# lxd99/TPNet

Measured on NVIDIA B200. Metric: temporal edges/sec (update+pairwise encode), higher is better.
Workload: dtype f32

## Files before the change

tpnet_b200/csrc/tpn_update.cu:

```cuda
#include <stdlib.h>

#include "tpn_common.cuh"
#include "tpn_radix.cuh"

namespace tpn {

namespace {

int g_debug_flags = 0;
thread_local int g_dev_slot = 0;

constexpr int kSmallMaxMsgs = 4096;
constexpr int kRankMaxMsgs = 1024;
constexpr int kPrepThreads = 1024;
constexpr int kWalkThreads = 256;
constexpr int kHubMin = 64;
constexpr int kGiantMin = 2048;
constexpr int kHubConsumers = 4;
constexpr int kHubThreads = (kHubConsumers + 1) * 32;
constexpr int kHubStages = 4;
constexpr int kHubSlotFloats = kHubConsumers * 32;
constexpr int kHubMetaChunk = 512;
constexpr int kChunkMin = 256;
constexpr size_t kSnapMaxBytes = (size_t)8 << 30;
constexpr int kSmallWalkThreads = 256;
constexpr int kHub2Producers = 7;
constexpr int kHub2Threads = (1 + kHub2Producers) * 32;
constexpr int kHub2SlotFloats = 64;
#ifndef TPN_HUB2_GIANT_FLOATS
#define TPN_HUB2_GIANT_FLOATS 16
#endif
constexpr int kHub2GiantFloats = TPN_HUB2_GIANT_FLOATS;
static_assert(kHub2GiantFloats == 8 || kHub2GiantFloats == 16 || kHub2GiantFloats == 32, "giant slices are 32, 64 or 128 bytes");
constexpr int kGiantLs = kHub2GiantFloats == 8 ? 1 : (kHub2GiantFloats == 16 ? 2 : 3);
constexpr int kGiantSpm = 16 >> kGiantLs;
constexpr int kGiantSpmMax = kGiantSpm > 4 ? kGiantSpm : 4;
constexpr int kHub2Stages = kHub2Producers + 4;
constexpr int kCtrGiant = 0, kCtrHub = 1, kCtrWork0 = 2, kCtrSmall = 6, kCtrHub2Work = 7, kCtrHub2Giant = 8;
constexpr int kCtrChunks = 9;
constexpr int kCtrStream = 10, kCtrStreamBlocks = 11, kCtrStreamProd = 12, kCtrStreamActive = 13, kCtrStreamChain = 14, kCtrStreamTicket = 15;
constexpr int kStreamSlice = kHub2GiantFloats;
constexpr int kStreamBlock = 32 * kGiantSpm;
constexpr uint32_t kNoPart = 0xffffffffu;
constexpr int kCtrSmClaim = 16;
constexpr int kCtrSlots = kCtrSmClaim + 256;
constexpr int kBarWords = 32;

struct DecayArgs {
    float c[TPN_MAX_LAYERS];
    int has_decay;
};

constexpr uint32_t kDirect = 0x80000000u;

struct MsgSource {
    const long long* a;
    const long long* b;
    const double* t;
    long long B;
    long long direct_from;
    __device__ __forceinline__ void get(int m, long long& tgt, long long& oth, int& widx) const {
        if (B > 0) {
            const int j = m < B ? m : (int)(m - B);
            tgt = m < B ? a[j] : b[j];
            oth = m < B ? b[j] : a[j];
            widx = j;
        } else {
            tgt = a[m];
            oth = b[m];
            widx = m;
        }
    }
};

struct Workspace {
    float* w;
    uint32_t* key_a;
    uint32_t* key_b;
    uint32_t* val_a;
    uint32_t* val_b;
    uint32_t* ssrc;
    float* sw;
    uint32_t* hist;
    uint32_t* hist2;
    uint32_t* bar;
    uint32_t* sslot;
    uint32_t* slen;
    float* snap;
    uint32_t* hub_giant;
    uint32_t* hub_reg;
    uint32_t* ctr;
    uint32_t* small_heads;
    uint32_t* hub_len;
    uint32_t* hub_part;
    uint32_t* giant_cbase;
    float* partial;
    int* svst;
    float* gprod;
    uint32_t* gflag;
    uint32_t* gblk;
    bool has_snap;
    bool has_stream;
    size_t bytes;
};

inline size_t snap_bytes(size_t E, int num_layer, int64_t row_stride) {
    return sizeof(float) * E * (size_t)num_layer * (size_t)row_stride;
}

inline size_t align_up(size_t x, size_t a) { return (x + a - 1) / a * a; }

constexpr size_t kStreamMaxBytes = (size_t)4 << 30;
constexpr int kGiantSortMaxC = 2048;
inline int stream_slices(int num_layer, int64_t row_stride) {
    return num_layer * (int)((row_stride + kStreamSlice - 1) / kStreamSlice);
}
inline size_t stream_prod_bytes(size_t E, int num_layer, int64_t row_stride) {
    return sizeof(float) * E * (size_t)stream_slices(num_layer, row_stride) * kStreamSlice + 256;
}
inline size_t stream_flag_words(size_t E) { return E / kStreamBlock + E / kGiantMin + 4; }

Workspace carve(void* base, int64_t batch, int num_layer, int64_t row_stride) {
    const size_t E = 2 * (size_t)batch;
    const size_t nblk = (E + kRadixTile - 1) / kRadixTile;
    char* p = reinterpret_cast<char*>(base);
    size_t off = 0;
    Workspace ws;
    auto take = [&](size_t bytes) { char* r = p ? p + off : nullptr; off += align_up(bytes, 256); return r; };
    ws.w = reinterpret_cast<float*>(take(sizeof(float) * E));
    ws.key_a = reinterpret_cast<uint32_t*>(take(4 * E));
    ws.key_b = reinterpret_cast<uint32_t*>(take(4 * E));
    ws.val_a = reinterpret_cast<uint32_t*>(take(4 * E));
    ws.val_b = reinterpret_cast<uint32_t*>(take(4 * E));
    ws.ssrc = reinterpret_cast<uint32_t*>(take(4 * E));
    ws.sw = reinterpret_cast<float*>(take(4 * E));
    ws.hist = reinterpret_cast<uint32_t*>(take(4 * kRadixBins * (nblk + 1)));
    ws.hist2 = reinterpret_cast<uint32_t*>(take(4 * kRadixBins * (nblk + 1)));
    ws.bar = reinterpret_cast<uint32_t*>(take(4 * kBarWords));
    ws.sslot = reinterpret_cast<uint32_t*>(take(4 * E));
    ws.slen = reinterpret_cast<uint32_t*>(take(4 * E));
    ws.has_snap = snap_bytes(E, num_layer, row_stride) <= kSnapMaxBytes;
    ws.snap = reinterpret_cast<float*>(take((ws.has_snap ? snap_bytes(E, num_layer, row_stride) : 0) + 16));
    ws.hub_giant = reinterpret_cast<uint32_t*>(take(4 * (E / kGiantMin + 2)));
    const size_t hub_cap = E / kHubMin + E / kChunkMin + E / kGiantMin + 4;
    const size_t part_rows = E / kChunkMin + E / kGiantMin + 2;
    ws.hub_reg = reinterpret_cast<uint32_t*>(take(4 * hub_cap));
    ws.hub_len = reinterpret_cast<uint32_t*>(take(4 * hub_cap));
    ws.hub_part = reinterpret_cast<uint32_t*>(take(4 * hub_cap));
    ws.giant_cbase = reinterpret_cast<uint32_t*>(take(4 * (E / kGiantMin + 2)));
    ws.partial = reinterpret_cast<float*>(take(ws.has_snap ? 4 * part_rows * (size_t)num_layer * (size_t)row_stride : 16));
    ws.ctr = reinterpret_cast<uint32_t*>(take(4 * kCtrSlots));
    ws.small_heads = reinterpret_cast<uint32_t*>(take(4 * E));
    ws.svst = reinterpret_cast<int*>(take(4 * (E + 4) * (size_t)(num_layer > 1 ? num_layer - 1 : 1) + 16));
    ws.gflag = reinterpret_cast<uint32_t*>(take(4 * stream_flag_words(E)));
    ws.gblk = reinterpret_cast<uint32_t*>(take(4 * (kGiantSortMaxC + 1)));
    ws.has_stream = ws.has_snap && stream_prod_bytes(E, num_layer, row_stride) <= kStreamMaxBytes &&
                    E / kGiantMin + 2 <= (size_t)kGiantSortMaxC;
    ws.gprod = reinterpret_cast<float*>(take(ws.has_stream ? stream_prod_bytes(E, num_layer, row_stride) : 16));
    ws.bytes = off;
    return ws;
}

__device__ __forceinline__ float edge_weight(double t, float t_last_f, float neg_lambda) {
    const float diff = __fsub_rn(t_last_f, (float)t);
    const float arg = __fmul_rn(neg_lambda, diff);
    return (float)exp((double)arg);
}

struct SweepArgs {
    long long total4;
    int ds4;
};

__device__ __forceinline__ void sweep_body(const StateView& st, const DecayArgs& decay, long long total4, int ds4,
                                           long long first, long long stride) {
    const long long per_node4 = (long long)st.num_layer * ds4;
    for (long long i = first; i < total4; i += stride) {
        const long long node = i / per_node4;
        const int r = (int)(i - node * per_node4);
        const int li = r / ds4;
        float* p = st.data + node * st.node_stride + st.row_stride + (long long)r * 4;
        float4 x = ld4(p);
        scale4(x, decay.c[li]);
        st4(p, x);
    }
}

__global__ void __launch_bounds__(kPrepThreads)
prep_small_kernel(MsgSource msgs, int E, float t_last_f, float neg_lambda, long long num_nodes,
                  uint32_t* __restrict__ skey, uint32_t* __restrict__ ssrc, float* __restrict__ sw,
                  uint32_t* __restrict__ sslot, uint32_t* __restrict__ slen, int* __restrict__ err_flag,
                  double* decay_log, int L, long long new_epoch, DecayArgs decay, StateView st, SweepArgs sweep) {
    if (blockIdx.x > 0) {
        sweep_body(st, decay, sweep.total4, sweep.ds4, (long long)(blockIdx.x - 1) * kPrepThreads + threadIdx.x,
                   (long long)(gridDim.x - 1) * kPrepThreads);
        return;
    }
    __shared__ __align__(16) unsigned long long comp[kSmallMaxMsgs];
    __shared__ float wsm[kSmallMaxMsgs];
    const int n_w = msgs.B > 0 ? (int)msgs.B : E;
    const bool message_mode = msgs.B == 0;
    const bool lazy = decay_log != nullptr;
    if (threadIdx.x == 0 && decay_log != nullptr && decay.has_decay) {
        for (int l = 0; l < L; ++l) decay_log[new_epoch * L + l] = decay_log[(new_epoch - 1) * L + l] * (double)decay.c[l];
    }
    if (E <= kRankMaxMsgs) {
        uint32_t* c32 = reinterpret_cast<uint32_t*>(comp);
        const bool narrow = num_nodes < (1ll << 22);
        const int Epad = (E + 3) & ~3;
        for (int m = threadIdx.x; m < Epad; m += kPrepThreads) {
            uint32_t key = 0xffffffffu >> 10;
            if (m < E) {
                long long tgt, oth;
                int widx;
                msgs.get(m, tgt, oth, widx);
                const bool ok = tgt >= 0 && tgt < num_nodes && oth >= 0 && oth < num_nodes;
                if (!ok && err_flag != nullptr) *err_flag = 1;
                key = ok ? (uint32_t)tgt : (uint32_t)num_nodes;
                if (m < n_w) wsm[m] = edge_weight(msgs.t[m], t_last_f, neg_lambda);
            }
            if (narrow) c32[m] = (key << 10) | (uint32_t)m;
            else comp[m] = ((unsigned long long)(m < E ? key : 0xffffffffu) << 32) | (uint32_t)m;
        }
// ... 42 lines not shown
            sw[rank] = wsm[j];
            sslot[rank] = (uint32_t)slot;
            slen[rank] = (uint32_t)(upper - lower);
        }
        return;
    }
    int P = 1;
    while (P < E) P <<= 1;
    for (int m = threadIdx.x; m < P; m += kPrepThreads) {
        unsigned long long c = ~0ull;
        if (m < E) {
            long long tgt, oth;
            int widx;
            msgs.get(m, tgt, oth, widx);
            const bool ok = tgt >= 0 && tgt < num_nodes && oth >= 0 && oth < num_nodes;
            if (!ok && err_flag != nullptr) *err_flag = 1;
            const uint32_t key = ok ? (uint32_t)tgt : (uint32_t)num_nodes;
            c = ((unsigned long long)key << 32) | (uint32_t)m;
            if (m < n_w) wsm[m] = edge_weight(msgs.t[m], t_last_f, neg_lambda);
        }
        comp[m] = c;
    }
    __syncthreads();
    for (int k = 2; k <= P; k <<= 1) {
        for (int j = k >> 1; j > 0; j >>= 1) {
            for (int i = threadIdx.x; i < P; i += kPrepThreads) {
                const int ixj = i ^ j;
                if (ixj > i) {
                    const unsigned long long a = comp[i], b = comp[ixj];
                    const bool up = (i & k) == 0;
                    if ((a > b) == up) { comp[i] = b; comp[ixj] = a; }
                }
            }
            __syncthreads();
        }
    }
    for (int p = threadIdx.x; p < E; p += kPrepThreads) {
        const unsigned long long c = comp[p];
        const uint32_t m = (uint32_t)c;
        const uint32_t mykey = (uint32_t)(c >> 32);
        long long tgt_unused, oth;
        int j;
        msgs.get((int)m, tgt_unused, oth, j);
        const uint32_t other = (uint32_t)oth;
        skey[p] = mykey;
        ssrc[p] = other;
        sw[p] = wsm[j];
        const unsigned long long other_lo = (unsigned long long)other << 32;
        const unsigned long long next_lo = (unsigned long long)(mykey + 1) << 32;
        int lo = 0, hi = E;
        while (lo < hi) {
            const int mid = (lo + hi) >> 1;
            if (comp[mid] < other_lo) lo = mid + 1; else hi = mid;
        }
        uint32_t slot = (uint32_t)lo;
        if (message_mode && (lo >= E || (uint32_t)(comp[lo] >> 32) != other)) {
            if (lazy && (long long)other < msgs.direct_from && err_flag != nullptr) *err_flag = 2;
            slot = kDirect;
        }
        sslot[p] = slot;
        lo = p; hi = E;
        while (lo < hi) {
            const int mid = (lo + hi) >> 1;
            if (comp[mid] < next_lo) lo = mid + 1; else hi = mid;
        }
        slen[p] = (uint32_t)(lo - p);
    }
}

struct PrepArgs {
    MsgSource msgs;
    Count count;
    float t_last_f, neg_lambda;
    long long num_nodes;
    float* w;
    uint32_t* key;
    uint32_t* val;
    int* err_flag;
    double* decay_log;
    int L;
    long long new_epoch;
    DecayArgs decay;
    uint32_t* ctr;
};

__device__ __forceinline__ void prep_body(const PrepArgs& a, int m) {
    if (m == 0 && a.decay_log != nullptr && a.decay.has_decay) {
        for (int l = 0; l < a.L; ++l)
            a.decay_log[a.new_epoch * a.L + l] = a.decay_log[(a.new_epoch - 1) * a.L + l] * (double)a.decay.c[l];
    }
    if (m < kCtrSlots) a.ctr[m] = 0;
    if (m == 0 && a.count.dev != nullptr && *a.count.dev > a.count.cap && a.err_flag != nullptr) *a.err_flag = 4;
    const int E = a.count.get();
    if (m >= E) return;
    long long tgt, oth;
    int widx;
    a.msgs.get(m, tgt, oth, widx);
    const bool ok = tgt >= 0 && tgt < a.num_nodes && oth >= 0 && oth < a.num_nodes;
    if (!ok && a.err_flag != nullptr) *a.err_flag = 1;
    const int n_w = a.msgs.B > 0 ? (int)a.msgs.B : E;
    if (m < n_w) a.w[m] = edge_weight(a.msgs.t[m], a.t_last_f, a.neg_lambda);
    a.key[m] = ok ? (uint32_t)tgt : (uint32_t)a.num_nodes;
    a.val[m] = (uint32_t)m;
}

__global__ void __launch_bounds__(256) prep_large_kernel(PrepArgs a) {
    prep_body(a, blockIdx.x * blockDim.x + threadIdx.x);
}

struct PayloadArgs {
    const uint32_t* order;
    const uint32_t* skey;
    uint32_t* key_out;
    MsgSource msgs;
    const float* w;
    Count count;
    uint32_t* ssrc;
    float* sw;
    uint32_t* sslot;
    uint32_t* slen;
    uint32_t* hub_giant;
    uint32_t* hub_reg;
    uint32_t* small_heads;
    uint32_t* ctr;
    int* svst;
    const int* stamps;
    int L, E4;
    long long num_nodes;
    int* err_flag;
    uint32_t* hub_len;
    uint32_t* hub_part;
    uint32_t* giant_cbase;
    int chunk;
};

__device__ __forceinline__ void payload_body(const PayloadArgs& a, int p) {
    const uint32_t* __restrict__ order = a.order;
    const uint32_t* __restrict__ skey = a.skey;
    const MsgSource& msgs = a.msgs;
    const float* __restrict__ w = a.w;
    const int E = a.count.get();
    uint32_t* __restrict__ ssrc = a.ssrc;
    float* __restrict__ sw = a.sw;
    uint32_t* __restrict__ sslot = a.sslot;
    uint32_t* __restrict__ slen = a.slen;
    uint32_t* __restrict__ hub_giant = a.hub_giant;
    uint32_t* __restrict__ hub_reg = a.hub_reg;
    uint32_t* __restrict__ small_heads = a.small_heads;
    uint32_t* __restrict__ ctr = a.ctr;
    int* __restrict__ svst = a.svst;
    const int* __restrict__ stamps = a.stamps;
    const int L = a.L, E4 = a.E4;
    const long long num_nodes = a.num_nodes;
    int* __restrict__ err_flag = a.err_flag;
    const int lane = threadIdx.x & 31;
    bool small_head = false;
    if (p < E) {
        const uint32_t m = order[p];
        long long tgt_unused, oth;
        int j;
        msgs.get((int)m, tgt_unused, oth, j);
        const uint32_t other = (uint32_t)oth;
        const uint32_t mykey = skey[p];
        if (a.key_out != skey) a.key_out[p] = mykey;
        ssrc[p] = other;
        float wv = w[j];
        if (sslot != nullptr) {
            int lo = 0, hi = E;
            while (lo < hi) {
                const int mid = (lo + hi) >> 1;
                if (skey[mid] < other) lo = mid + 1; else hi = mid;
            }
            uint32_t slot = (uint32_t)lo;
            if (msgs.B == 0 && (lo >= E || skey[lo] != other)) {
                if (stamps != nullptr && (long long)other < msgs.direct_from && err_flag != nullptr) *err_flag = 2;
                slot = kDirect;
                wv = __int_as_float(__float_as_int(wv) | 0x80000000);
            }
            sslot[p] = slot;
        }
        sw[p] = wv;
        uint32_t len = 0;
        if (p == 0 || skey[p - 1] != mykey) {
            int lo = p, hi = E;
            while (lo < hi) {
                const int mid = (lo + hi) >> 1;
                if (skey[mid] <= mykey) lo = mid + 1; else hi = mid;
            }
            len = (uint32_t)(lo - p);
            if ((long long)mykey < num_nodes) {
                if (len >= (uint32_t)kGiantMin) {
                    const uint32_t gi = atomicAdd(&ctr[kCtrGiant], 1u);
                    hub_giant[gi] = (uint32_t)p;
                    if (a.chunk > 0) {
                        const uint32_t nch = (len + (uint32_t)a.chunk - 1u) / (uint32_t)a.chunk;
                        const uint32_t cb = atomicAdd(&ctr[kCtrChunks], nch);
                        const uint32_t eb = atomicAdd(&ctr[kCtrHub], nch);
                        a.giant_cbase[gi] = cb;
                        for (uint32_t c = 0; c < nch; ++c) {
                            hub_reg[eb + c] = (uint32_t)p + c * (uint32_t)a.chunk;
                            a.hub_len[eb + c] = min((uint32_t)a.chunk, len - c * (uint32_t)a.chunk);
                            a.hub_part[eb + c] = cb + c;
                        }
                    }
                } else if (len >= (uint32_t)kHubMin) {
                    const uint32_t e = atomicAdd(&ctr[kCtrHub], 1u);
                    hub_reg[e] = (uint32_t)p;
                    a.hub_len[e] = len;
                    a.hub_part[e] = kNoPart;
                } else {
                    small_head = true;
                }
            }
        }
        slen[p] = len;
        if (svst != nullptr) {
            for (int l = 0; l < L - 1; ++l)
                svst[(size_t)l * E4 + p] = (long long)other < num_nodes ? stamps[(long long)other * L + l] : -1;
        }
    }
    const uint32_t mask = __ballot_sync(0xffffffffu, small_head);
    if (mask != 0) {
        const int leader = __ffs(mask) - 1;
        uint32_t base = 0;
        if (lane == leader) base = atomicAdd(&ctr[kCtrSmall], (uint32_t)__popc(mask));
        base = __shfl_sync(0xffffffffu, base, leader);
        if (small_head) small_heads[base + __popc(mask & ((1u << lane) - 1u))] = (uint32_t)p;
    }
}

__global__ void __launch_bounds__(256) payload_kernel(PayloadArgs a) {
    payload_body(a, blockIdx.x * blockDim.x + threadIdx.x);
}

constexpr int kGiantSortMax = kGiantSortMaxC;
struct GiantSmem {
    uint32_t head_s[kGiantSortMax], len_s[kGiantSortMax], sorted_s[kGiantSortMax];
};
__device__ __forceinline__ void sort_giants_body(GiantSmem& sm, uint32_t* __restrict__ hub_giant,
                                                 const uint32_t* __restrict__ slen, uint32_t* __restrict__ ctr,
                                                 uint32_t* __restrict__ gblk, uint32_t* __restrict__ gflag, Count count,
                                                 int stream_mode) {
    const uint32_t stream_min = stream_mode == 0 ? 0u
                                : (stream_mode == 2 ? (uint32_t)kGiantMin
                                                    : max((uint32_t)kGiantMin, (uint32_t)(count.get() >> 2)));
    const int n = (int)ctr[kCtrGiant];
    if (n < 1 || n > kGiantSortMax) return;
    for (int i = threadIdx.x; i < n; i += blockDim.x) {
        sm.head_s[i] = hub_giant[i];
        sm.len_s[i] = slen[sm.head_s[i]];
    }
    __syncthreads();
    for (int i = threadIdx.x; i < n; i += blockDim.x) {
        const uint32_t li = sm.len_s[i];
        int rank = 0;
        for (int j = 0; j < n; ++j) rank += (sm.len_s[j] > li || (sm.len_s[j] == li && j < i)) ? 1 : 0;
        hub_giant[rank] = sm.head_s[i];
        sm.sorted_s[rank] = li;
    }
    __syncthreads();
    if (threadIdx.x == 0 && stream_min > 0) {
        uint32_t blocks = 0;
        int ns = 0;
        for (; ns < n && sm.sorted_s[ns] >= stream_min; ++ns) {
            gblk[ns] = blocks;
            blocks += (sm.sorted_s[ns] + (uint32_t)kStreamBlock - 1u) / (uint32_t)kStreamBlock;
        }
        gblk[ns] = blocks;
        ctr[kCtrStream] = (uint32_t)ns;
        ctr[kCtrStreamBlocks] = blocks;
        sm.head_s[0] = blocks;
    }
    __syncthreads();
    if (stream_min > 0) {
        const uint32_t blocks = sm.head_s[0];
        for (uint32_t i = threadIdx.x; i < blocks; i += blockDim.x) gflag[i] = 0;
    }
}
__global__ void __launch_bounds__(1024)
sort_giants_kernel(uint32_t* __restrict__ hub_giant, const uint32_t* __restrict__ slen, uint32_t* __restrict__ ctr,
                   uint32_t* __restrict__ gblk, uint32_t* __restrict__ gflag, Count count, int stream_mode) {
    __shared__ GiantSmem sm;
    sort_giants_body(sm, hub_giant, slen, ctr, gblk, gflag, count, stream_mode);
}

struct FrontArgs {
    PrepArgs prep;
    uint32_t *key_a, *key_b, *val_a, *val_b, *hist, *hist2, *bar;
    int passes;
};

__device__ __forceinline__ void grid_barrier(uint32_t* bar, uint32_t& target, int* err_flag) {
    __syncthreads();
    if (threadIdx.x == 0) {
        target += gridDim.x;
        __threadfence();
        atomicAdd(bar, 1u);
        uint32_t seen;
        long long spins = 0;
        do {
            asm volatile("ld.acquire.gpu.global.u32 %0, [%1];" : "=r"(seen) : "l"(bar) : "memory");
            if (seen >= target) break;
            if (++spins > (1ll << 22)) {
                if (err_flag != nullptr) *err_flag = 8;
                break;
            }
        } while (true);
    }
    __syncthreads();
}

union FrontSmem {
    uint32_t bins[kRadixBins];
    ScatterSmem scatter;
};
// ... 93 lines not shown

    float* tbase = st.data + (long long)key * st.node_stride + (long long)(ALL ? 1 : layer) * st.row_stride;
    float4 acc[V];
#pragma unroll
    for (int k = 0; k < V; ++k) {
        const int c = col0 + k * 32;
        const int tli = ALL ? (c < span4 ? c / ds4 : 0) : layer - 1;
        long long tstamp = 0;
        if (LAZY && c < span4) tstamp = st.stamps[(long long)key * L + tli];
        acc[k] = (c < span4 && tstamp >= 0) ? ld4(tbase + 4 * (long long)c) : make_float4(0.f, 0.f, 0.f, 0.f);
        if (LAZY && c < span4 && tstamp >= 0) scale4(acc[k], decay_factor(st, tli, tstamp));
    }

    for (int base = 0; base < len; base += 32) {
        const int nmsg = min(32, len - base);
        uint32_t my_v = 0, my_slot = 0;
        float my_w = 0.f;
        long long my_vstamp = 0;
        if (lane < nmsg) {
            const int p = wid + base + lane;
            my_v = ssrc[p];
            my_w = sw[p];
            if (ALL) my_slot = sslot[p];
            else if (LAZY && layer >= 2) my_vstamp = st.stamps[(long long)my_v * L + (layer - 2)];
        }
        for (int j0 = 0; j0 < nmsg; j0 += D) {
            float4 x[D][V];
            float w[D];
            long long vstamp[D];
#pragma unroll
            for (int j = 0; j < D; ++j) {
                const int jj = j0 + j;
                const int sl = jj < nmsg ? jj : 0;
                const uint32_t v = __shfl_sync(0xffffffffu, my_v, sl);
                w[j] = __shfl_sync(0xffffffffu, my_w, sl);
                const uint32_t slot = ALL ? __shfl_sync(0xffffffffu, my_slot, sl) : 0u;
                vstamp[j] = (!ALL && LAZY) ? __shfl_sync(0xffffffffu, my_vstamp, sl) : 0;
                const float* sstate = st.data + (long long)v * st.node_stride +
                                      (long long)(ALL ? 0 : layer - 1) * st.row_stride;
                const bool direct = ALL && (slot & kDirect) != 0;
                const float* ssnap = ALL ? snap + (long long)(slot & ~kDirect) * snap4 * 4 : nullptr;
#pragma unroll
                for (int k = 0; k < V; ++k) {
                    const int c = col0 + k * 32;
                    float4 val = make_float4(0.f, 0.f, 0.f, 0.f);
                    if (jj < nmsg && c < span4) {
                        if (ALL) {
                            val = (c < soff || direct) ? ld4(sstate + 4 * (long long)c)
                                                       : ld4(ssnap + 4 * (long long)(c - soff));
                            if (LAZY && direct && c >= ds4) {
                                const int sli = c / ds4 - 1;
                                const int sst = st.stamps[(long long)v * L + sli];
                                if (sst >= 0) scale4(val, decay_factor(st, sli, sst));
                            }
                        }
                        else if (vstamp[j] >= 0) val = ld4(sstate + 4 * (long long)c);
                    }
                    x[j][k] = val;
                }
            }
#pragma unroll
            for (int j = 0; j < D; ++j) {
                if (j0 + j < nmsg) {
                    if (!ALL && LAZY && layer >= 2 && vstamp[j] >= 0) {
                        const float f = decay_factor(st, layer - 2, vstamp[j]);
#pragma unroll
                        for (int k = 0; k < V; ++k) scale4(x[j][k], f);
                    }
#pragma unroll
                    for (int k = 0; k < V; ++k) axpy4_rn(acc[k], x[j][k], w[j]);
                }
            }
        }
    }
#pragma unroll
    for (int k = 0; k < V; ++k) {
        const int c = col0 + k * 32;
        if (c < span4) st4(tbase + 4 * (long long)c, acc[k]);
    }
    if (LAZY && write_stamp && lane == 0) st.stamps[(long long)key * L + (layer - 1)] = (int)st.epoch;
}

template <bool LAZY>
__global__ void __launch_bounds__(256)
snapshot_kernel(StateView st, const uint32_t* __restrict__ skey, Count count, int ds4, float* __restrict__ snap,
                int srow0) {
    const int p = (blockIdx.x * 256 + threadIdx.x) >> 5;
    const int lane = threadIdx.x & 31;
    if (p >= count.get()) return;
    const uint32_t key = skey[p];
    if ((long long)key >= st.num_nodes) return;
    if (p > 0 && skey[p - 1] == key) return;
    const int L = st.num_layer;
    const int snap4 = (L - srow0) * ds4;
    const float* rows = st.data + (long long)key * st.node_stride + (long long)srow0 * st.row_stride;
    float* slot = snap + (long long)p * snap4 * 4;
    float fmine = 1.0f;
    if (LAZY && lane < L - srow0 && srow0 + lane >= 1) {
        const int li = srow0 + lane - 1;
        const long long stamp = st.stamps[(long long)key * L + li];
        fmine = stamp >= 0 ? decay_factor(st, li, stamp) : -1.0f;
    }
    float f[TPN_MAX_LAYERS];
#pragma unroll
    for (int l = 0; l < TPN_MAX_LAYERS; ++l) f[l] = LAZY ? __shfl_sync(0xffffffffu, fmine, l) : 1.0f;
    for (int c0 = lane; c0 < snap4; c0 += 128) {
        float4 v[4];
        float fk[4];
#pragma unroll
        for (int k = 0; k < 4; ++k) {
            const int c = c0 + 32 * k;
            const int li = c / ds4;
            fk[k] = li == 0 ? f[0] : (li == 1 ? f[1] : (li == 2 ? f[2] : f[3]));
            v[k] = (c < snap4 && fk[k] >= 0.f) ? ld4(rows + 4 * (long long)c) : make_float4(0.f, 0.f, 0.f, 0.f);
        }
#pragma unroll
        for (int k = 0; k < 4; ++k) {
            const int c = c0 + 32 * k;
            if (c < snap4) {
                if (LAZY && fk[k] >= 0.f && fk[k] != 1.0f) scale4(v[k], fk[k]);
                st4(slot + 4 * (long long)c, v[k]);
            }
        }
    }
}

__global__ void __launch_bounds__(256)
stamp_targets_kernel(StateView st, int layer, const uint32_t* __restrict__ skey, Count count) {
    const int p = blockIdx.x * blockDim.x + threadIdx.x;
    if (p >= count.get()) return;
    const uint32_t key = skey[p];
    if ((long long)key >= st.num_nodes) return;
    if (p > 0 && skey[p - 1] == key) return;
    if (layer >= 1) {
        st.stamps[(long long)key * st.num_layer + (layer - 1)] = (int)st.epoch;
    } else {
        for (int l = 0; l < st.num_layer; ++l) st.stamps[(long long)key * st.num_layer + l] = (int)st.epoch;
    }
}


struct HubSmem {
    float ring[kHubStages][32][kHubSlotFloats];
    float wring[kHubStages][32];
    int vring[kHubStages][32];
    uint32_t msrc[2][kHubMetaChunk + 4];
    float mw[2][kHubMetaChunk + 4];
    uint32_t mx[2][kHubMetaChunk + 4];
    uint64_t full[kHubStages];
    uint64_t empty[kHubStages];
    uint64_t mfull[2];
    int item[4];
};

template <bool LAZY, bool ALL>
__global__ void __launch_bounds__(kHubThreads)
walk_hub_kernel(StateView st, int layer, const uint32_t* __restrict__ skey, const uint32_t* __restrict__ ssrc,
                const float* __restrict__ sw, const uint32_t* __restrict__ xarr, const uint32_t* __restrict__ slen,
                const float* __restrict__ snap, const uint32_t* __restrict__ hub_giant,
                const uint32_t* __restrict__ hub_reg, uint32_t* __restrict__ ctr, int work_ctr, int span,
                int slice_w, int slices, DecayArgs dnow) {
    extern __shared__ __align__(128) unsigned char hub_raw[];
    HubSmem& sm = *reinterpret_cast<HubSmem*>(hub_raw);
    const int warp = threadIdx.x >> 5;
    const int lane = threadIdx.x & 31;
    const int L = st.num_layer;
    const int rs = (int)st.row_stride;
    const bool has_x = ALL || (LAZY && layer >= 2);
    if (threadIdx.x == 0) {
        for (int i = 0; i < kHubStages; ++i) {
            mbar_init(&sm.full[i], 1);
            mbar_init(&sm.empty[i], kHubConsumers);
        }
        mbar_init(&sm.mfull[0], 1);
        mbar_init(&sm.mfull[1], 1);
        asm volatile("fence.mbarrier_init.release.cluster;" ::: "memory");
    }
    __syncthreads();
    const uint32_t n_giant = ctr[0], n_reg = ctr[1];
    const uint32_t total = (n_giant + n_reg) * (uint32_t)slices;
    uint32_t blk = 0;
    uint32_t mit = 0;
    for (;;) {
        if (threadIdx.x == 0) sm.item[0] = (int)atomicAdd(&ctr[work_ctr], 1u);
        __syncthreads();
        const uint32_t work = (uint32_t)sm.item[0];
        __syncthreads();
        if (work >= total) break;
        const uint32_t it = work / (uint32_t)slices;
        const int slice = (int)(work - it * (uint32_t)slices);
        const int head = (int)(it < n_giant ? hub_giant[it] : hub_reg[it - n_giant]);
        const int len = (int)slen[head];
        const uint32_t key = skey[head];
        const int c0 = slice * slice_w;
        const int c1 = min(span, c0 + slice_w);
        const uint32_t msg_bytes = (uint32_t)(c1 - c0) * 4u;

        if (warp == kHubConsumers) {
            const int nchunk = (len + kHubMetaChunk - 1) / kHubMetaChunk;
            auto issue_meta = [&](int c, uint32_t m) {
                const int cs = c * kHubMetaChunk;
                const int cn = min(kHubMetaChunk, len - cs);
                const int a0 = (head + cs) & ~3;
                const uint32_t bytes = (uint32_t)(((head + cs + cn) - a0 + 3) & ~3) * 4u;
                const int buf = (int)(m & 1u);
                fence_proxy_async_smem();
// ... 1040 lines not shown
    const bool lazy = st->stamps != nullptr;
    const int L = st->num_layer;

    DecayArgs dargs;
    dargs.has_decay = 0;
    for (int l = 0; l < TPN_MAX_LAYERS; ++l) dargs.c[l] = 1.0f;
    if (decay != nullptr) {
        bool all_one = true;
        for (int l = 0; l < L; ++l) {
            dargs.c[l] = decay[l];
            all_one = all_one && decay[l] == 1.0f;
        }
        dargs.has_decay = all_one ? 0 : 1;
    }
    long long new_epoch = st->epoch;
    double new_floor = st->cum_floor;
    if (lazy && dargs.has_decay) {
        if (st->epoch + 1 >= st->log_capacity) return TPN_ERR_LOG_FULL;
        double cmin = 1.0;
        for (int l = 0; l < L; ++l) cmin = dargs.c[l] < cmin ? (double)dargs.c[l] : cmin;
        new_floor = (st->epoch == 0 ? 1.0 : st->cum_floor);
        if (st->epoch > 0 && !(new_floor * cmin >= 1e-200)) return TPN_ERR_LOG_FULL;
        new_floor *= cmin;
        new_epoch = st->epoch + 1;
    }

    const int ds4 = (int)(st->row_stride / 4);
    const float t_last_f = (float)t_last;
    double* log_w = lazy ? st->decay_log : nullptr;
    const bool force_per_layer = (g_debug_flags & TPN_DEBUG_PER_LAYER_WALK) != 0;
    const bool snapshot_path = ws.has_snap && !(force_per_layer && !(count_dev == nullptr && E <= kSmallMaxMsgs));
    const bool small_path = count_dev == nullptr && E <= kSmallMaxMsgs;
    const bool hubs = !small_path;
    const int E4 = (E + 3) & ~3;
    const bool eager_sweep = !lazy && dargs.has_decay;
    int chunk = st->giant_chunk > 0 ? (int)st->giant_chunk : 0;
    if (chunk > 0 && chunk < kChunkMin) chunk = kChunkMin;
    if (chunk > kGiantMin) chunk = kGiantMin;
    chunk &= ~31;
    const long long sweep_total4 = st->num_nodes * (long long)L * ds4;
    const int stream_mode = (ws.has_stream && chunk == 0 && (g_debug_flags & TPN_DEBUG_NO_STREAM) == 0)
                                ? ((g_debug_flags & TPN_DEBUG_STREAM_ALL) ? 2 : 1) : 0;

    StateView view = make_view(st);
    view.epoch = new_epoch;

    const bool do_front = phase != TPN_UPDATE_APPLY;
    const bool do_rest = phase != TPN_UPDATE_PREPARE;
    const bool snap_early = lazy && !small_path;
    if (small_path) {
        if (phase == TPN_UPDATE_PREPARE) return TPN_OK;
        SweepArgs sw_args;
        sw_args.total4 = eager_sweep ? sweep_total4 : 0;
        sw_args.ds4 = ds4;
        unsigned grid = 1;
        if (eager_sweep) {
            const long long want = (sweep_total4 + kPrepThreads - 1) / kPrepThreads;
            const long long cap = (long long)device_sm_count() * 4;
            grid += (unsigned)(want < cap ? (want < 1 ? 1 : want) : cap);
        }
        prep_small_kernel<<<grid, kPrepThreads, 0, stream>>>(msgs, E, t_last_f, neg_lambda, st->num_nodes, ws.key_a,
                                                             ws.ssrc, ws.sw, ws.sslot, ws.slen, err_flag_dev, log_w, L,
                                                             new_epoch, dargs, view, sw_args);
    } else if (do_front) {
        int bits = 0;
        while ((1ll << bits) <= st->num_nodes) ++bits;
        const int passes = (bits + 7) / 8;
        const int nblk = (E + kRadixTile - 1) / kRadixTile;
        struct { PrepArgs prep; PayloadArgs pay; } fa;
        fa.prep.msgs = msgs;
        fa.prep.count = cnt;
        fa.prep.t_last_f = t_last_f;
        fa.prep.neg_lambda = neg_lambda;
        fa.prep.num_nodes = st->num_nodes;
        fa.prep.w = ws.w;
        fa.prep.key = ws.key_a;
        fa.prep.val = ws.val_a;
        fa.prep.err_flag = err_flag_dev;
        fa.prep.decay_log = log_w;
        fa.prep.L = L;
        fa.prep.new_epoch = new_epoch;
        fa.prep.decay = dargs;
        fa.prep.ctr = ws.ctr;
        fa.pay.order = nullptr;
        fa.pay.skey = nullptr;
        fa.pay.key_out = ws.key_a;
        fa.pay.msgs = msgs;
        fa.pay.w = ws.w;
        fa.pay.count = cnt;
        fa.pay.ssrc = ws.ssrc;
        fa.pay.sw = ws.sw;
        fa.pay.sslot = snapshot_path ? ws.sslot : nullptr;
        fa.pay.slen = ws.slen;
        fa.pay.hub_giant = ws.hub_giant;
        fa.pay.hub_reg = ws.hub_reg;
        fa.pay.small_heads = ws.small_heads;
        fa.pay.ctr = ws.ctr;
        fa.pay.svst = (lazy && !snapshot_path && L >= 2) ? ws.svst : nullptr;
        fa.pay.stamps = st->stamps;
        fa.pay.L = L;
        fa.pay.E4 = E4;
        fa.pay.num_nodes = st->num_nodes;
        fa.pay.err_flag = err_flag_dev;
        fa.pay.hub_len = ws.hub_len;
        fa.pay.hub_part = ws.hub_part;
        fa.pay.giant_cbase = ws.giant_cbase;
        fa.pay.chunk = (snapshot_path && hubs) ? chunk : 0;
        const bool fused_front = (g_debug_flags & TPN_DEBUG_LEGACY_FRONT) == 0 && front_kernel_ok();
        if (fused_front) {
            FrontArgs fr;
            fr.prep = fa.prep;
            fr.key_a = ws.key_a; fr.key_b = ws.key_b; fr.val_a = ws.val_a; fr.val_b = ws.val_b;
            fr.hist = ws.hist; fr.hist2 = ws.hist2; fr.bar = ws.bar;
            fr.passes = passes;
            const int sms = device_sm_count();
            const unsigned grid = (unsigned)(nblk < 1 ? 1 : (nblk < sms ? nblk : sms));
            void* kargs[] = {&fr};
            if (cudaMemsetAsync(ws.bar, 0, 4 * kBarWords, stream) != cudaSuccess ||
                cudaLaunchCooperativeKernel((const void*)front_kernel, dim3(grid), dim3(kRadixThreads), kargs, 0,
                                            stream) != cudaSuccess) {
                set_cuda_error(cudaGetLastError());
                return TPN_ERR_CUDA;
            }
            const bool odd = (passes & 1) != 0;
            fa.pay.order = odd ? ws.val_b : ws.val_a;
            fa.pay.skey = odd ? ws.key_b : ws.key_a;
            payload_kernel<<<(E + 255) / 256, 256, 0, stream>>>(fa.pay);
            if (snapshot_path && chunk == 0) {
                sort_giants_kernel<<<1, 1024, 0, stream>>>(ws.hub_giant, ws.slen, ws.ctr, ws.gblk, ws.gflag, cnt, stream_mode);
            }
        } else
        {
            prep_large_kernel<<<(unsigned)((E + 255) / 256 < 2 ? 2 : (E + 255) / 256), 256, 0, stream>>>(fa.prep);
            uint32_t *kin = ws.key_a, *kout = ws.key_b, *vin = ws.val_a, *vout = ws.val_b;
            for (int p = 0; p < passes; ++p) {
                radix_hist_kernel<<<nblk, kRadixThreads, 0, stream>>>(kin, cnt, 8 * p, ws.hist);
                const int prefixed = (nblk > kRadixDirectBlocks || count_dev != nullptr) ? 1 : 0;
                if (prefixed) radix_prefix_kernel<<<kRadixBins / 8, 256, 0, stream>>>(ws.hist, cnt);
                radix_scatter_kernel<<<nblk, kRadixThreads, 0, stream>>>(kin, vin, kout, vout, cnt, 8 * p, ws.hist,
                                                                         prefixed);
                uint32_t* tk = kin; kin = kout; kout = tk;
                uint32_t* tv = vin; vin = vout; vout = tv;
            }
            fa.pay.order = vin;
            fa.pay.skey = kin;
            payload_kernel<<<(E + 255) / 256, 256, 0, stream>>>(fa.pay);
            if (snapshot_path && chunk == 0) {
                sort_giants_kernel<<<1, 1024, 0, stream>>>(ws.hub_giant, ws.slen, ws.ctr, ws.gblk, ws.gflag, cnt, stream_mode);
            }
        }
    }
    if (!small_path && do_rest && eager_sweep) {
        const long long want = (sweep_total4 + 255) / 256;
        const long long cap = (long long)device_sm_count() * 16;
        const unsigned grid = (unsigned)(want < cap ? (want < 1 ? 1 : want) : cap);
        sweep_decay_kernel<<<grid, 256, 0, stream>>>(view, dargs, sweep_total4, ds4);
    }

    const int srow0 = (g_debug_flags & TPN_DEBUG_SNAPSHOT_P0) ? 0 : 1;
    if (snapshot_path) {
        if (L - srow0 >= 1 && (snap_early ? do_front : do_rest)) {
            const unsigned grid = (unsigned)(((long long)E * 32 + 255) / 256);
            if (lazy) snapshot_kernel<true><<<grid, 256, 0, stream>>>(view, ws.key_a, cnt, ds4, ws.snap, srow0);
            else snapshot_kernel<false><<<grid, 256, 0, stream>>>(view, ws.key_a, cnt, ds4, ws.snap, srow0);
        }
        if (!do_rest) {
        } else if (hubs) {
            const bool direct = msgs.B == 0;
            SideStream* side = (g_debug_flags & TPN_DEBUG_SERIAL_WALK) ? nullptr : side_stream();
            cudaStream_t hub_stream = stream, giant_stream = stream;
            if (side != nullptr) {
                if (cudaEventRecord(side->fork, stream) == cudaSuccess &&
                    cudaStreamWaitEvent(side->stream, side->fork, 0) == cudaSuccess) {
                    hub_stream = side->stream;
                    if (stream_mode > 0 && cudaStreamWaitEvent(side->stream2, side->fork, 0) == cudaSuccess)
                        giant_stream = side->stream2;
                } else {
                    (void)cudaGetLastError();
                }
            }
            if (stream_mode > 0) {
                const int src = direct ? launch_walk_stream<true>(view, ws, lazy, srow0, err_flag_dev, giant_stream)
                                       : launch_walk_stream<false>(view, ws, lazy, srow0, err_flag_dev, giant_stream);
                if (src != TPN_OK) return src;
            }
            const int hrc = direct ? launch_walk_hub2<true>(view, ws, lazy, dargs, chunk, srow0, hub_stream)
                                   : launch_walk_hub2<false>(view, ws, lazy, dargs, chunk, srow0, hub_stream);
            if (hrc != TPN_OK) return hrc;
            if (direct) launch_walk_small<true>(view, ws, E, ds4, lazy, dargs, srow0, stream);
            else launch_walk_small<false>(view, ws, E, ds4, lazy, dargs, srow0, stream);
            if (hub_stream != stream) {
                bool ok = cudaEventRecord(side->join, hub_stream) == cudaSuccess &&
                          cudaStreamWaitEvent(stream, side->join, 0) == cudaSuccess;
                if (giant_stream != stream)
                    ok = ok && cudaEventRecord(side->join2, giant_stream) == cudaSuccess &&
                         cudaStreamWaitEvent(stream, side->join2, 0) == cudaSuccess;
                if (!ok) {
                    set_cuda_error(cudaGetLastError());
                    return TPN_ERR_CUDA;
                }
            }
        } else {
            const int span4 = L * ds4;
            launch_walk<1, 16, true>(view, 0, ws, cnt, ds4, (span4 + 31) / 32, lazy, false, dargs, stream, srow0);
        }
        if (lazy && do_rest) stamp_targets_kernel<<<(E + 255) / 256, 256, 0, stream>>>(view, 0, ws.key_a, cnt);
    } else if (do_rest) {
        int vpl = (ds4 + 31) / 32;
        int tiles = 1;
        if (vpl > 4) {
            tiles = (vpl + 3) / 4;
            vpl = 4;
        }
        for (int layer = L; layer >= 1; --layer) {
            if (hubs) {
                const int hrc = launch_walk_hub<false>(view, layer, ws, E4, lazy, dargs, stream);
                if (hrc != TPN_OK) return hrc;
            }
            switch (vpl) {
                case 1: launch_walk<1, 16, false>(view, layer, ws, cnt, ds4, tiles, lazy, hubs, dargs, stream); break;
                case 2: launch_walk<2, 8, false>(view, layer, ws, cnt, ds4, tiles, lazy, hubs, dargs, stream); break;
                case 3: launch_walk<3, 4, false>(view, layer, ws, cnt, ds4, tiles, lazy, hubs, dargs, stream); break;
                default: launch_walk<4, 4, false>(view, layer, ws, cnt, ds4, tiles, lazy, hubs, dargs, stream); break;
            }
            if (lazy && (tiles > 1 || hubs))
                stamp_targets_kernel<<<(E + 255) / 256, 256, 0, stream>>>(view, layer, ws.key_a, cnt);
        }
    }
    const int lrc = check_launch();
    if (lrc == TPN_OK && do_rest) {
        st->epoch = new_epoch;
        st->cum_floor = new_floor;
    }
    return lrc;
}

}
}

#ifdef TPN_HUB2_TIMELINE
extern "C" int tpn_debug_hub_timeline(unsigned long long* host_out, size_t count) {
    const size_t have = sizeof(tpn::g_hub2_timeline) / sizeof(unsigned long long);
    if (host_out == nullptr || count > have) return TPN_ERR_INVALID_ARGUMENT;
    return cudaMemcpyFromSymbol(host_out, tpn::g_hub2_timeline, count * sizeof(unsigned long long)) == cudaSuccess
               ? TPN_OK : TPN_ERR_CUDA;
}
#endif
// ... 76 lines not shown
```

Measured before the change: 160.3 million.

## Replace binary searches with hash table of run heads and compact snapshot walk

Adds a heads kernel that compacts the start position of each distinct sorted key into a list and inserts it into an open-addressing hash table. The payload kernel then finds source slots and run lengths by hash lookup instead of binary search over the sorted keys, with run lengths computed at each run's tail. The snapshot kernel becomes a grid-stride loop over the compact head list with a capped grid and launch bounds, rather than one warp per edge. The price is an extra kernel launch, table clearing in prep and atomic CAS insertion. Snapshot slots are now indexed by head ordinal instead of sorted position, so every consumer of the snapshot must agree on that indexing.

```diff
diff --git a/tpnet_b200/csrc/tpn_update.cu b/tpnet_b200/csrc/tpn_update.cu
--- a/tpnet_b200/csrc/tpn_update.cu
+++ b/tpnet_b200/csrc/tpn_update.cu
@@ -42,7 +42,8 @@
 constexpr int kStreamSlice = kHub2GiantFloats;
 constexpr int kStreamBlock = 32 * kGiantSpm;
 constexpr uint32_t kNoPart = 0xffffffffu;
-constexpr int kCtrSmClaim = 16;
+constexpr int kCtrHeads = 16;
+constexpr int kCtrSmClaim = 17;
 constexpr int kCtrSlots = kCtrSmClaim + 256;
 constexpr int kBarWords = 32;
 
@@ -52,6 +53,29 @@
 };
 
 constexpr uint32_t kDirect = 0x80000000u;
+
+constexpr unsigned long long kHeadEmpty = ~0ull;
+constexpr uint32_t kNoSlot = 0xffffffffu;
+__host__ __device__ __forceinline__ int head_table_bits(long long E) {
+    int b = 2;
+    while ((1ll << b) < 2 * E) ++b;
+    return b;
+}
+__device__ __forceinline__ uint32_t head_hash(uint32_t key, int bits) { return (key * 2654435761u) >> (32 - bits); }
+__device__ __forceinline__ void head_insert(unsigned long long* tab, int bits, uint32_t key, uint32_t slot) {
+    const uint32_t mask = (1u << bits) - 1u;
+    const unsigned long long e = ((unsigned long long)key << 32) | slot;
+    for (uint32_t h = head_hash(key, bits);; h = (h + 1u) & mask)
+        if (atomicCAS(&tab[h], kHeadEmpty, e) == kHeadEmpty) return;
+}
+__device__ __forceinline__ uint32_t head_find(const unsigned long long* tab, int bits, uint32_t key) {
+    const uint32_t mask = (1u << bits) - 1u;
+    for (uint32_t h = head_hash(key, bits);; h = (h + 1u) & mask) {
+        const unsigned long long e = tab[h];
+        if (e == kHeadEmpty) return kNoSlot;
+        if ((uint32_t)(e >> 32) == key) return (uint32_t)e;
+    }
+}
 
 struct MsgSource {
     const long long* a;
@@ -86,6 +110,8 @@
     uint32_t* bar;
     uint32_t* sslot;
     uint32_t* slen;
+    uint2* hlist;
+    unsigned long long* htab;
     float* snap;
     uint32_t* hub_giant;
     uint32_t* hub_reg;
@@ -139,6 +165,8 @@
     ws.bar = reinterpret_cast<uint32_t*>(take(4 * kBarWords));
     ws.sslot = reinterpret_cast<uint32_t*>(take(4 * E));
     ws.slen = reinterpret_cast<uint32_t*>(take(4 * E));
+    ws.hlist = reinterpret_cast<uint2*>(take(8 * E));
+    ws.htab = reinterpret_cast<unsigned long long*>(take(8 * ((size_t)1 << head_table_bits((long long)E))));
     ws.has_snap = snap_bytes(E, num_layer, row_stride) <= kSnapMaxBytes;
     ws.snap = reinterpret_cast<float*>(take((ws.has_snap ? snap_bytes(E, num_layer, row_stride) : 0) + 16));
     ws.hub_giant = reinterpret_cast<uint32_t*>(take(4 * (E / kGiantMin + 2)));
@@ -347,6 +375,7 @@
     long long new_epoch;
     DecayArgs decay;
     uint32_t* ctr;
+    unsigned long long* htab;
 };
 
 __device__ __forceinline__ void prep_body(const PrepArgs& a, int m) {
@@ -358,6 +387,10 @@
     if (m == 0 && a.count.dev != nullptr && *a.count.dev > a.count.cap && a.err_flag != nullptr) *a.err_flag = 4;
     const int E = a.count.get();
     if (m >= E) return;
+    if (4ll * m < (1ll << head_table_bits(E))) {
+        reinterpret_cast<ulonglong2*>(a.htab)[2 * m] = make_ulonglong2(kHeadEmpty, kHeadEmpty);
+        reinterpret_cast<ulonglong2*>(a.htab)[2 * m + 1] = make_ulonglong2(kHeadEmpty, kHeadEmpty);
+    }
     long long tgt, oth;
     int widx;
     a.msgs.get(m, tgt, oth, widx);
@@ -397,6 +430,8 @@
     uint32_t* hub_part;
     uint32_t* giant_cbase;
     int chunk;
+    const uint2* hlist;
+    const unsigned long long* htab;
 };
 
 __device__ __forceinline__ void payload_body(const PayloadArgs& a, int p) {
@@ -420,6 +455,7 @@
     int* __restrict__ err_flag = a.err_flag;
     const int lane = threadIdx.x & 31;
     bool small_head = false;
+    uint32_t small_pos = 0;
     if (p < E) {
         const uint32_t m = order[p];
         long long tgt_unused, oth;
@@ -429,15 +465,12 @@
         const uint32_t mykey = skey[p];
         if (a.key_out != skey) a.key_out[p] = mykey;
         ssrc[p] = other;
+        const int hbits = head_table_bits(E);
         float wv = w[j];
         if (sslot != nullptr) {
-            int lo = 0, hi = E;
-            while (lo < hi) {
-                const int mid = (lo + hi) >> 1;
-                if (skey[mid] < other) lo = mid + 1; else hi = mid;
-            }
-            uint32_t slot = (uint32_t)lo;
-            if (msgs.B == 0 && (lo >= E || skey[lo] != other)) {
+            uint32_t slot = head_find(a.htab, hbits, other);
+            if (slot == kNoSlot && msgs.B > 0) slot = 0;
+            if (slot == kNoSlot) {
                 if (stamps != nullptr && (long long)other < msgs.direct_from && err_flag != nullptr) *err_flag = 2;
                 slot = kDirect;
                 wv = __int_as_float(__float_as_int(wv) | 0x80000000);
@@ -445,40 +478,36 @@
             sslot[p] = slot;
         }
         sw[p] = wv;
-        uint32_t len = 0;
-        if (p == 0 || skey[p - 1] != mykey) {
-            int lo = p, hi = E;
-            while (lo < hi) {
-                const int mid = (lo + hi) >> 1;
-                if (skey[mid] <= mykey) lo = mid + 1; else hi = mid;
-            }
-            len = (uint32_t)(lo - p);
-            if ((long long)mykey < num_nodes) {
-                if (len >= (uint32_t)kGiantMin) {
-                    const uint32_t gi = atomicAdd(&ctr[kCtrGiant], 1u);
-                    hub_giant[gi] = (uint32_t)p;
-                    if (a.chunk > 0) {
-                        const uint32_t nch = (len + (uint32_t)a.chunk - 1u) / (uint32_t)a.chunk;
-                        const uint32_t cb = atomicAdd(&ctr[kCtrChunks], nch);
-                        const uint32_t eb = atomicAdd(&ctr[kCtrHub], nch);
-                        a.giant_cbase[gi] = cb;
-                        for (uint32_t c = 0; c < nch; ++c) {
-                            hub_reg[eb + c] = (uint32_t)p + c * (uint32_t)a.chunk;
-                            a.hub_len[eb + c] = min((uint32_t)a.chunk, len - c * (uint32_t)a.chunk);
-                            a.hub_part[eb + c] = cb + c;
-                        }
+        if ((long long)mykey >= num_nodes) {
+            if (p == 0 || skey[p - 1] != mykey) slen[p] = (uint32_t)(E - p);
+        } else if (p == E - 1 || skey[p + 1] != mykey) {
+            const uint32_t head = a.hlist[head_find(a.htab, hbits, mykey)].y;
+            const uint32_t len = (uint32_t)p + 1u - head;
+            slen[head] = len;
+            if (len >= (uint32_t)kGiantMin) {
+                const uint32_t gi = atomicAdd(&ctr[kCtrGiant], 1u);
+                hub_giant[gi] = head;
+                if (a.chunk > 0) {
+                    const uint32_t nch = (len + (uint32_t)a.chunk - 1u) / (uint32_t)a.chunk;
+                    const uint32_t cb = atomicAdd(&ctr[kCtrChunks], nch);
+                    const uint32_t eb = atomicAdd(&ctr[kCtrHub], nch);
+                    a.giant_cbase[gi] = cb;
+                    for (uint32_t c = 0; c < nch; ++c) {
+                        hub_reg[eb + c] = head + c * (uint32_t)a.chunk;
+                        a.hub_len[eb + c] = min((uint32_t)a.chunk, len - c * (uint32_t)a.chunk);
+                        a.hub_part[eb + c] = cb + c;
                     }
-                } else if (len >= (uint32_t)kHubMin) {
-                    const uint32_t e = atomicAdd(&ctr[kCtrHub], 1u);
-                    hub_reg[e] = (uint32_t)p;
-                    a.hub_len[e] = len;
-                    a.hub_part[e] = kNoPart;
-                } else {
-                    small_head = true;
-                }
-            }
-        }
-        slen[p] = len;
+                }
+            } else if (len >= (uint32_t)kHubMin) {
+                const uint32_t e = atomicAdd(&ctr[kCtrHub], 1u);
+                hub_reg[e] = head;
+                a.hub_len[e] = len;
+                a.hub_part[e] = kNoPart;
+            } else {
+                small_head = true;
+                small_pos = head;
+            }
+        }
         if (svst != nullptr) {
             for (int l = 0; l < L - 1; ++l)
                 svst[(size_t)l * E4 + p] = (long long)other < num_nodes ? stamps[(long long)other * L + l] : -1;
@@ -490,12 +519,37 @@
         uint32_t base = 0;
         if (lane == leader) base = atomicAdd(&ctr[kCtrSmall], (uint32_t)__popc(mask));
         base = __shfl_sync(0xffffffffu, base, leader);
-        if (small_head) small_heads[base + __popc(mask & ((1u << lane) - 1u))] = (uint32_t)p;
+        if (small_head) small_heads[base + __popc(mask & ((1u << lane) - 1u))] = small_pos;
     }
 }
 
 __global__ void __launch_bounds__(256) payload_kernel(PayloadArgs a) {
     payload_body(a, blockIdx.x * blockDim.x + threadIdx.x);
+}
+
+__global__ void __launch_bounds__(256)
+heads_kernel(const uint32_t* __restrict__ skey, Count count, long long num_nodes, uint2* __restrict__ hlist,
+             unsigned long long* __restrict__ htab, uint32_t* __restrict__ ctr) {
+    const int p = blockIdx.x * blockDim.x + threadIdx.x;
+    const int lane = threadIdx.x & 31;
+    const int E = count.get();
+    uint32_t key = 0;
+    bool head = false;
+    if (p < E) {
+        key = skey[p];
+        head = (long long)key < num_nodes && (p == 0 || skey[p - 1] != key);
+    }
+    const uint32_t mask = __ballot_sync(0xffffffffu, head);
+    if (mask == 0) return;
+    const int leader = __ffs(mask) - 1;
+    uint32_t base = 0;
+    if (lane == leader) base = atomicAdd(&ctr[kCtrHeads], (uint32_t)__popc(mask));
+    base = __shfl_sync(0xffffffffu, base, leader);
+    if (head) {
+        const uint32_t s = base + __popc(mask & ((1u << lane) - 1u));
+        hlist[s] = make_uint2(key, (uint32_t)p);
+        head_insert(htab, head_table_bits(E), key, s);
+    }
 }
 
 constexpr int kGiantSortMax = kGiantSortMaxC;
@@ -755,19 +809,11 @@
 }
 
 template <bool LAZY>
-__global__ void __launch_bounds__(256)
-snapshot_kernel(StateView st, const uint32_t* __restrict__ skey, Count count, int ds4, float* __restrict__ snap,
-                int srow0) {
-    const int p = (blockIdx.x * 256 + threadIdx.x) >> 5;
-    const int lane = threadIdx.x & 31;
-    if (p >= count.get()) return;
-    const uint32_t key = skey[p];
-    if ((long long)key >= st.num_nodes) return;
-    if (p > 0 && skey[p - 1] == key) return;
+__device__ __forceinline__ void snapshot_row(const StateView& st, uint32_t key, int ds4, float* __restrict__ slot,
+                                             int srow0, int lane) {
     const int L = st.num_layer;
     const int snap4 = (L - srow0) * ds4;
     const float* rows = st.data + (long long)key * st.node_stride + (long long)srow0 * st.row_stride;
-    float* slot = snap + (long long)p * snap4 * 4;
     float fmine = 1.0f;
     if (LAZY && lane < L - srow0 && srow0 + lane >= 1) {
         const int li = srow0 + lane - 1;
@@ -795,6 +841,27 @@
                 st4(slot + 4 * (long long)c, v[k]);
             }
         }
+    }
+}
+
+constexpr int kSnapCtasPerSm = 5;
+template <bool LAZY>
+__global__ void __launch_bounds__(256, kSnapCtasPerSm)
+snapshot_kernel(StateView st, const uint2* __restrict__ hlist, const uint32_t* __restrict__ ctr,
+                const uint32_t* __restrict__ skey, Count count, int ds4, float* __restrict__ snap, int srow0) {
+    const int lane = threadIdx.x & 31;
+    const int n = hlist != nullptr ? (int)ctr[kCtrHeads] : count.get();
+    const int snap4 = (st.num_layer - srow0) * ds4;
+    const int nwarps = (int)(gridDim.x * blockDim.x) >> 5;
+    for (int i = (int)(blockIdx.x * blockDim.x + threadIdx.x) >> 5; i < n; i += nwarps) {
+        uint32_t key;
+        if (hlist != nullptr) {
+            key = hlist[i].x;
+        } else {
+            key = skey[i];
+            if ((long long)key >= st.num_nodes || (i > 0 && skey[i - 1] == key)) continue;
+        }
+        snapshot_row<LAZY>(st, key, ds4, snap + (long long)i * snap4 * 4, srow0, lane);
     }
 }
 
@@ -2001,6 +2068,7 @@
         fa.prep.new_epoch = new_epoch;
         fa.prep.decay = dargs;
         fa.prep.ctr = ws.ctr;
+        fa.prep.htab = ws.htab;
         fa.pay.order = nullptr;
         fa.pay.skey = nullptr;
         fa.pay.key_out = ws.key_a;
@@ -2025,6 +2093,8 @@
         fa.pay.hub_part = ws.hub_part;
         fa.pay.giant_cbase = ws.giant_cbase;
         fa.pay.chunk = (snapshot_path && hubs) ? chunk : 0;
+        fa.pay.hlist = ws.hlist;
+        fa.pay.htab = ws.htab;
         const bool fused_front = (g_debug_flags & TPN_DEBUG_LEGACY_FRONT) == 0 && front_kernel_ok();
         if (fused_front) {
             FrontArgs fr;
@@ -2044,6 +2114,7 @@
             const bool odd = (passes & 1) != 0;
             fa.pay.order = odd ? ws.val_b : ws.val_a;
             fa.pay.skey = odd ? ws.key_b : ws.key_a;
+            heads_kernel<<<(E + 255) / 256, 256, 0, stream>>>(fa.pay.skey, cnt, st->num_nodes, ws.hlist, ws.htab, ws.ctr);
             payload_kernel<<<(E + 255) / 256, 256, 0, stream>>>(fa.pay);
             if (snapshot_path && chunk == 0) {
                 sort_giants_kernel<<<1, 1024, 0, stream>>>(ws.hub_giant, ws.slen, ws.ctr, ws.gblk, ws.gflag, cnt, stream_mode);
@@ -2063,6 +2134,7 @@
             }
             fa.pay.order = vin;
             fa.pay.skey = kin;
+            heads_kernel<<<(E + 255) / 256, 256, 0, stream>>>(kin, cnt, st->num_nodes, ws.hlist, ws.htab, ws.ctr);
             payload_kernel<<<(E + 255) / 256, 256, 0, stream>>>(fa.pay);
             if (snapshot_path && chunk == 0) {
                 sort_giants_kernel<<<1, 1024, 0, stream>>>(ws.hub_giant, ws.slen, ws.ctr, ws.gblk, ws.gflag, cnt, stream_mode);
@@ -2079,9 +2151,12 @@
     const int srow0 = (g_debug_flags & TPN_DEBUG_SNAPSHOT_P0) ? 0 : 1;
     if (snapshot_path) {
         if (L - srow0 >= 1 && (snap_early ? do_front : do_rest)) {
-            const unsigned grid = (unsigned)(((long long)E * 32 + 255) / 256);
-            if (lazy) snapshot_kernel<true><<<grid, 256, 0, stream>>>(view, ws.key_a, cnt, ds4, ws.snap, srow0);
-            else snapshot_kernel<false><<<grid, 256, 0, stream>>>(view, ws.key_a, cnt, ds4, ws.snap, srow0);
+            const long long want = ((long long)E * 32 + 255) / 256;
+            const long long cap = (long long)device_sm_count() * kSnapCtasPerSm;
+            const unsigned grid = (unsigned)(want < cap ? want : cap);
+            const uint2* hl = small_path ? nullptr : ws.hlist;
+            if (lazy) snapshot_kernel<true><<<grid, 256, 0, stream>>>(view, hl, ws.ctr, ws.key_a, cnt, ds4, ws.snap, srow0);
+            else snapshot_kernel<false><<<grid, 256, 0, stream>>>(view, hl, ws.ctr, ws.key_a, cnt, ds4, ws.snap, srow0);
         }
         if (!do_rest) {
         } else if (hubs) {
```

Measured after the change: 164.5 million (median of 6 runs). +2.6%, better.
